# raulmur/ORB_SLAM2

Measured on NVIDIA H100. Metric: stereo frames/sec (ORB extract L+R + ComputeStereoMatches, KITTI-shaped 1242x375 @2000 kpts), higher is better.
Workload: dtype u8

## Files before the change

orb_slam2_b200/csrc/borb_host.cu:

```cuda
#include <cmath>
#include <cstdarg>
#include <cstdio>
#include <algorithm>
#include <cstdlib>
#include <cstring>

#include "borb_internal.h"

namespace borb {

static thread_local std::string tl_error;
void set_error(const char* fmt, ...) {
    char buf[512];
    va_list ap;
    va_start(ap, fmt);
    vsnprintf(buf, sizeof(buf), fmt, ap);
    va_end(ap);
    tl_error = buf;
}

std::atomic<int> g_poison{-1};

bool allow_max_smem(const void* func) {
    static std::mutex mu;
// ... 30 lines not shown
    e->per_level.assign(L, 0);
    const float factor = (float)(1.0 / sf);
    float want = (float)e->cfg.n_features * (1.f - factor) / (1.f - (float)std::pow((double)factor, (double)L));
    int sum = 0;
    for (int l = 0; l < L - 1; l++) {
        e->per_level[l] = cv_round_f(want);
        sum += e->per_level[l];
        want *= factor;
    }
    e->per_level[L - 1] = e->cfg.n_features - sum > 0 ? e->cfg.n_features - sum : 0;
    const int vmax = (int)std::floor(HALF_PATCH * std::sqrt(2.f) / 2 + 1);
    const int vmin = (int)std::ceil(HALF_PATCH * std::sqrt(2.f) / 2);
    for (int v = 0; v < 16; v++) e->umax[v] = 0;
    for (int v = 0; v <= vmax; ++v) e->umax[v] = (int)lrint(std::sqrt((double)HALF_PATCH * HALF_PATCH - (double)v * v));
    for (int v = HALF_PATCH, v0 = 0; v >= vmin; --v) {
        while (e->umax[v0] == e->umax[v0 + 1]) ++v0;
        e->umax[v] = v0;
        ++v0;
    }
}

void resize_table(int src, int dst, bool clamp_edges, int extra, std::vector<int16_t>& out) {
    const double inv = (double)dst / src, scale = 1. / inv;
    const size_t first = out.size();
    for (int d = 0; d < dst; d++) {
        float f = (float)((d + 0.5) * scale - 0.5);
        int s = (int)std::floor(f);
        f -= s;
        if (clamp_edges) {
            if (s < 0) { f = 0; s = 0; }
            if (s >= src - 1) { f = 0; s = src - 1; }
        }
        out.push_back((int16_t)s);
        out.push_back((int16_t)cv_round_f((1.f - f) * 2048.f));
        out.push_back((int16_t)cv_round_f(f * 2048.f));
        out.push_back(0);
    }
    for (int k = 0; k < extra; k++) {
        int r = 2 * dst - 2 - (dst + k);
        if (r < 0) r = 0;
        for (int j = 0; j < 4; j++) out.push_back(out[first + (size_t)r * 4 + j]);
    }
    if (((out.size() - first) / 4) & 1) for (int j = 0; j < 4; j++) out.push_back(0);
}

bool resize_window_table(const std::vector<int16_t>& tabs, size_t xtab_first, int n_entries, std::vector<int16_t>& out) {
    bool ok = true;
    for (int gq = 0; gq < n_entries; gq += 4) {
        int lo = 1 << 30, hi = 0;
        for (int i = 0; i < 4; i++) {
            const int ofs = tabs[xtab_first + (size_t)(gq + i) * 4];
            lo = std::min(lo, ofs); hi = std::max(hi, ofs);
        }
        const int base = lo & ~3;
        if (hi + 1 - base > 11) ok = false;
        for (int i = 0; i < 4; i++) {
            const int16_t* e = &tabs[xtab_first + (size_t)(gq + i) * 4];
            const int pos = e[0] - base;
            int s1 = 0, s2 = 0x10;
            if (pos <= 6) s1 = pos | ((pos + 1) << 4);
            else if (pos == 7) { s1 = 7; s2 = 0x40; }
            else { const int q = (pos - 8) + 4; s2 = q | ((q + 1) << 4); }
            out.push_back(e[1]);
            out.push_back(e[2]);
            out.push_back((int16_t)base);
            out.push_back((int16_t)((s1 | (s2 << 8)) & 0x7FFF));
        }
    }
    return ok;
}

const int8_t kPattern[1024] = {
#include "orb_pattern.inc"
};

borb_status build_geometry(borb_extractor* e, int w, int h, std::vector<int16_t>& tabs) {
    Geometry& g = e->geom;
    std::memset(&g, 0, sizeof(g));
    const int L = e->cfg.n_levels;
    g.nlevels = L; g.w = w; g.h = h;
    g.fast_mode = e->fast_mode;
    g.ini_th = e->cfg.ini_th_fast;
    g.min_th = e->cfg.min_th_fast;
    for (int i = 0; i < 16; i++) g.umax[i] = e->umax[i];
    unsigned pyr_off = 0, cand_off = 0;
    int blk = 0, sel_off = 0, btile = 0;
    tabs.clear();
    for (int l = 0; l < L; l++) {
        LevelGeom& v = g.lv[l];
        v.w = cv_round_f((float)w * e->inv_scale[l]);
        v.h = cv_round_f((float)h * e->inv_scale[l]);
        const float width = (float)(v.w - 2 * MIN_BORDER), height = (float)(v.h - 2 * MIN_BORDER);
        v.nCols = (int)(width / 30.f);
        v.nRows = (int)(height / 30.f);
        if (v.nCols < 1 || v.nRows < 1) {
            set_error("level %d is %dx%d: too small for the 30-px FAST cell grid (reference divides by zero)", l, v.w, v.h);
            return BORB_ERR_UNSUPPORTED;
        }
        v.wCell = (int)std::ceil(width / v.nCols);
        v.hCell = (int)std::ceil(height / v.nRows);
        v.pitch = align_up(v.w + 8, 128);
        v.pyr_off = pyr_off;
        pyr_off += (unsigned)v.pitch * v.h;
        v.cellsPerBlk = FAST_TILE_W / v.wCell > 0 ? FAST_TILE_W / v.wCell : 1;
        v.rowsPerBlk = fast_rows_per_blk(v.nRows, v.hCell);
        v.blkCols = (v.nCols + v.cellsPerBlk - 1) / v.cellsPerBlk;
        v.blkBase = blk;
        blk += v.blkCols * ((v.nRows + v.rowsPerBlk - 1) / v.rowsPerBlk);
        v.cand_off = cand_off;
        v.cand_cap = v.nCols * v.nRows * ((v.wCell + 1) / 2) * ((v.hCell + 1) / 2);
        cand_off += (unsigned)align_up(v.cand_cap, 32);
        v.quota = e->per_level[l];
        v.nIni = (int)std::round(width / height);
        if (v.nIni < 1) { set_error("level %d aspect ratio gives zero quadtree roots (reference divides by zero)", l); return BORB_ERR_UNSUPPORTED; }
        v.hX = width / v.nIni;
        v.node_cap = (v.quota > 4 * v.nIni ? v.quota : 4 * v.nIni) + 3;
        v.node_cap = align_up(v.node_cap + 1, 4);
        v.sel_off = sel_off;
        sel_off += v.node_cap;
        v.scale = e->scale[l];
        v.inv_scale = e->inv_scale[l];
        v.patch_size = (float)(int)(PATCH * e->scale[l]);
        g.blur_base[l] = btile;
        btile += ((v.w + BLUR_TILE_W - 1) / BLUR_TILE_W) * ((v.h + BLUR_TILE_H - 1) / BLUR_TILE_H);
        if (l > 0) {
            const int wpad = (v.w + 8 + 3) & ~3;
            v.xtab_off = (unsigned)(tabs.size() / 4);
            resize_table(g.lv[l - 1].w, v.w, true, wpad - v.w, tabs);
            v.ytab_off = (unsigned)(tabs.size() / 4);
            resize_table(g.lv[l - 1].h, v.h, false, 0, tabs);
            v.xwin_off = (unsigned)(tabs.size() / 4);
            std::vector<int16_t> win;
            v.x_windowed = resize_window_table(tabs, (size_t)v.xtab_off * 4, wpad, win) ? 1 : 0;
            tabs.insert(tabs.end(), win.begin(), win.end());
        }
        if (quadtree_smem_bytes(v.node_cap) > 200 * 1024) {
            set_error("per-level quota %d exceeds the quadtree kernel's shared-memory envelope", v.quota);
            return BORB_ERR_UNSUPPORTED;
        }
    }
    g.blur_base[L] = btile;
    g.blur_tiles = btile;
    g.fast_blocks = blk;
    g.pyr_image_stride = (unsigned)align_up((int)pyr_off, g.lv[0].pitch);
    g.cand_image_stride = cand_off;
    g.sel_image_stride = sel_off;
    if (sel_off >= 65536) { set_error("keypoint capacity %d exceeds 65535", sel_off); return BORB_ERR_UNSUPPORTED; }
    return BORB_OK;
}

void free_workspace(Workspace& ws) {
    cudaFree(ws.pyr); cudaFree(ws.blur); cudaFree(ws.cand); cudaFree(ws.cand_cnt); cudaFree(ws.pnode); cudaFree(ws.sel);
    cudaFree(ws.sel_cnt); cudaFree(ws.kps); cudaFree(ws.desc); cudaFree(ws.nkp); cudaFree(ws.u_right); cudaFree(ws.depth);
    cudaFree(ws.sad); cudaFree(ws.tabs); cudaFree(ws.brief_slots); cudaFree(ws.pair_idx); cudaFree(ws.st_bins); cudaFree(ws.st_recs); cudaFree(ws.stage);
    free(ws.fast_tmaps); cudaFree(ws.fast_tiles);
    ws = Workspace();
}

borb_status ensure(borb_extractor* e, int w, int h, int n_images) {
    if (w < 1 || h < 1 || w > BORB_MAX_DIM || h > BORB_MAX_DIM) { set_error("image size %dx%d outside [1,%d]", w, h, BORB_MAX_DIM); return BORB_ERR_UNSUPPORTED; }
    BORB_CUDA(cudaSetDevice(e->device));
    const bool same_shape = e->have_geom && e->geom.w == w && e->geom.h == h;
    if (same_shape && e->ws.max_images >= n_images) return BORB_OK;
    BORB_CUDA(cudaStreamSynchronize(e->stream));
    std::vector<int16_t> tabs;
    e->have_geom = false;
    e->last_n_images = 0;
    e->last_stereo_pairs = 0;
    borb_status st = build_geometry(e, w, h, tabs);
    if (st != BORB_OK) return st;
    size_t n = (size_t)(n_images > 2 ? n_images : 2);
    if (same_shape && (size_t)e->ws.max_images > n) n = (size_t)e->ws.max_images;
    free_workspace(e->ws);
    if (e->h_counts) { cudaFreeHost(e->h_counts); e->h_counts = nullptr; }
    e->pair_cache.clear();
    const Geometry& g = e->geom;
    Workspace& ws = e->ws;
    BORB_CUDA(cudaMalloc(&ws.pyr, n * g.pyr_image_stride + 256));
    BORB_CUDA(cudaMalloc(&ws.blur, n * g.pyr_image_stride + 256));
    BORB_CUDA(cudaMalloc(&ws.cand, n * g.cand_image_stride * sizeof(uint32_t)));
    BORB_CUDA(cudaMalloc(&ws.pnode, n * g.cand_image_stride * sizeof(int)));
    BORB_CUDA(cudaMalloc(&ws.cand_cnt, n * g.nlevels * sizeof(int)));
    BORB_CUDA(cudaMalloc(&ws.sel, n * g.sel_image_stride * sizeof(uint32_t)));
    BORB_CUDA(cudaMalloc(&ws.sel_cnt, n * g.nlevels * sizeof(int)));
    BORB_CUDA(cudaMalloc(&ws.kps, n * g.sel_image_stride * sizeof(borb_keypoint)));
    BORB_CUDA(cudaMalloc(&ws.desc, n * g.sel_image_stride * 32));
    BORB_CUDA(cudaMalloc(&ws.nkp, n * sizeof(int)));
    BORB_CUDA(cudaMalloc(&ws.u_right, n * g.sel_image_stride * sizeof(float)));
    BORB_CUDA(cudaMalloc(&ws.depth, n * g.sel_image_stride * sizeof(float)));
    BORB_CUDA(cudaMalloc(&ws.sad, n * g.sel_image_stride * sizeof(int)));
    BORB_CUDA(cudaMalloc(&ws.pair_idx, n * 2 * sizeof(int)));
    BORB_CUDA(cudaMalloc(&ws.st_bins, n * stereo_bins_bytes_per_pair()));
    ws.st_recs_bytes = n * (size_t)stereo_rec_stride(g) * stereo_rec_bytes();
    BORB_CUDA(cudaMalloc(&ws.st_recs, ws.st_recs_bytes));
    BORB_CUDA(cudaMalloc(&ws.tabs, (tabs.size() + 4) * sizeof(int16_t)));
    BORB_CUDA(cudaMemcpy(ws.tabs, tabs.data(), tabs.size() * sizeof(int16_t), cudaMemcpyHostToDevice));
    const std::vector<uint32_t>& slots = brief_slot_table();
    BORB_CUDA(cudaMalloc(&ws.brief_slots, slots.size() * sizeof(uint32_t)));
    BORB_CUDA(cudaMemcpy(ws.brief_slots, slots.data(), slots.size() * sizeof(uint32_t), cudaMemcpyHostToDevice));
    BORB_CUDA(cudaMemset(ws.nkp, 0, n * sizeof(int)));
    BORB_CUDA(cudaMallocHost(&e->h_counts, n * 2 * sizeof(int)));
    ws.max_images = (int)n;
    ws.fast_tmaps = malloc(fast_tmaps_bytes());
    if ((st = build_fast_tmaps(g, ws, ws.fast_tmaps)) != BORB_OK) return st;
    if ((st = build_fast_tiles(g, ws)) != BORB_OK) return st;
    e->have_geom = true;
    return BORB_OK;
}

borb_status poison_extract(borb_extractor* e) {
    const int p = poison_byte();
    if (p < 0) return BORB_OK;
    const Geometry& g = e->geom;
    Workspace& ws = e->ws;
    const size_t n = (size_t)ws.max_images;
    cudaStream_t s = e->stream;
    if (ws.stage) BORB_CUDA(cudaMemsetAsync(ws.stage, p, ws.stage_bytes, s));
    BORB_CUDA(cudaMemsetAsync(ws.pyr, p, n * g.pyr_image_stride + 256, s));
    BORB_CUDA(cudaMemsetAsync(ws.blur, p, n * g.pyr_image_stride + 256, s));
    BORB_CUDA(cudaMemsetAsync(ws.cand, p, n * g.cand_image_stride * sizeof(uint32_t), s));
    BORB_CUDA(cudaMemsetAsync(ws.pnode, p, n * g.cand_image_stride * sizeof(int), s));
    BORB_CUDA(cudaMemsetAsync(ws.cand_cnt, p, n * g.nlevels * sizeof(int), s));
    BORB_CUDA(cudaMemsetAsync(ws.sel, p, n * g.sel_image_stride * sizeof(uint32_t), s));
    BORB_CUDA(cudaMemsetAsync(ws.sel_cnt, p, n * g.nlevels * sizeof(int), s));
    BORB_CUDA(cudaMemsetAsync(ws.kps, p, n * g.sel_image_stride * sizeof(borb_keypoint), s));
    BORB_CUDA(cudaMemsetAsync(ws.desc, p, n * g.sel_image_stride * 32, s));
    BORB_CUDA(cudaMemsetAsync(ws.nkp, p, n * sizeof(int), s));
    return BORB_OK;
}

borb_status poison_stereo(borb_extractor* e) {
    const int p = poison_byte();
    if (p < 0) return BORB_OK;
    Workspace& ws = e->ws;
    const size_t n = (size_t)ws.max_images * e->geom.sel_image_stride;
    cudaStream_t s = e->stream;
    BORB_CUDA(cudaMemsetAsync(ws.u_right, p, n * sizeof(float), s));
    BORB_CUDA(cudaMemsetAsync(ws.depth, p, n * sizeof(float), s));
    BORB_CUDA(cudaMemsetAsync(ws.sad, p, n * sizeof(int), s));
    BORB_CUDA(cudaMemsetAsync(ws.st_bins, p, (size_t)ws.max_images * stereo_bins_bytes_per_pair(), s));
    BORB_CUDA(cudaMemsetAsync(ws.st_recs, p, ws.st_recs_bytes, s));
    return BORB_OK;
}

void drain_timing(borb_extractor* e);
void begin_step(borb_extractor* e) {
    if (!e->timing) return;
    if (e->ev.empty()) {
        e->ev.resize((size_t)borb_extractor::EV_RING * 9);
        for (auto& x : e->ev) cudaEventCreate(&x);
    }
    if (e->ev_pending >= borb_extractor::EV_RING) {
        cudaStreamSynchronize(e->stream);
        drain_timing(e);
    }
    e->ev_slot = (e->ev_slot + 1) % borb_extractor::EV_RING;
    e->ev_mask[e->ev_slot] = 0;
    e->ev_pending++;
}
void mark(borb_extractor* e, int i) {
    if (!e->timing || e->ev.empty()) return;
    cudaEventRecord(e->ev[(size_t)e->ev_slot * 9 + i], e->stream);
    e->ev_mask[e->ev_slot] |= 1u << i;
}
void drain_timing(borb_extractor* e) {
    const int R = borb_extractor::EV_RING;
    for (int k = e->ev_pending - 1; k >= 0; k--) {
        const int slot = ((e->ev_slot - k) % R + R) % R;
        const unsigned m = e->ev_mask[slot];
        for (int i = 0; i < 8; i++) {
            float ms = 0.f;
            if (m & (1u << i)) {
                int j = i + 1;
                while (j < 9 && !(m & (1u << j))) j++;
                if (j < 9 && cudaEventElapsedTime(&ms, e->ev[(size_t)slot * 9 + i], e->ev[(size_t)slot * 9 + j]) != cudaSuccess) { ms = 0.f; cudaGetLastError(); }
            }
            e->stage_ms[i] = ms;
            e->stage_sum_ms[i] += ms;
        }
        e->stage_steps++;
    }
    e->ev_pending = 0;
}

borb_status enqueue_extract(borb_extractor* e, int n) {
    const Geometry& g = e->geom;
    Workspace& ws = e->ws;
    cudaStream_t s = e->stream;
    BORB_CUDA(cudaMemsetAsync(ws.cand_cnt, 0, (size_t)n * g.nlevels * sizeof(int), s));
    mark(e, 1);
    e->launches += launch_pyramid(g, ws, n, s);
    mark(e, 2);
    e->launches += launch_fast(g, ws, n, s);
    mark(e, 3);
    e->launches += launch_quadtree(g, ws, n, s);
    mark(e, 4);
    e->launches += launch_blur(g, ws, n, s);
    mark(e, 5);
    e->launches += launch_describe(g, ws, n, s);
    mark(e, 6);
    BORB_CUDA(cudaGetLastError());
    e->last_n_images = n;
    e->last_stereo_pairs = 0;
    return BORB_OK;
}

borb_status rectified_size(borb_extractor* e, int w, int h, int* gw, int* gh) {
    if (!e->d_map[0][0]) return BORB_OK;
    if (w != e->map_src_w || h != e->map_src_h) {
        set_error("rectification maps were built for %dx%d raw frames, got %dx%d", e->map_src_w, e->map_src_h, w, h);
        return BORB_ERR_INVALID_ARG;
    }
    *gw = e->map_dst_w; *gh = e->map_dst_h;
    return BORB_OK;
}

borb_status upload_slots(borb_extractor* e, const uint8_t* const* slots, int n, int w, int h, int stride, bool stereo_pairs = false) {
    const Geometry& g = e->geom;
    const int ch = e->in_channels;
    if (stride < w * ch) { set_error("stride %d smaller than a row of %d %d-channel pixels", stride, w, ch); return BORB_ERR_INVALID_ARG; }
    const size_t img_bytes = (size_t)stride * h;
    bool contiguous = n > 1 || ch > 1 || e->d_map[0][0] != nullptr;
    for (int k = 0; k < n; k++) {
        if (!slots[k]) { set_error("image %d is NULL", k); return BORB_ERR_INVALID_ARG; }
        if (slots[k] != slots[0] + (size_t)k * img_bytes) contiguous = false;
    }
    auto need_stage = [&](size_t need) -> borb_status {
        if (e->ws.stage_bytes < need) {
            BORB_CUDA(cudaStreamSynchronize(e->stream));
            cudaFree(e->ws.stage);
            e->ws.stage = nullptr; e->ws.stage_bytes = 0;
            BORB_CUDA(cudaMalloc(&e->ws.stage, need));
            e->ws.stage_bytes = need;
            if (poison_byte() >= 0) BORB_CUDA(cudaMemsetAsync(e->ws.stage, poison_byte(), need, e->stream));
        }
        return BORB_OK;
    };
    if (e->d_map[0][0]) {
        if (ch != 1) { set_error("rectification maps apply to CV_8UC1 frames"); return BORB_ERR_UNSUPPORTED; }
        const size_t src_img = contiguous ? img_bytes : (size_t)w * h;
        const int src_stride = contiguous ? stride : w;
        borb_status st = need_stage(src_img * n);
        if (st != BORB_OK) return st;
        if (contiguous) BORB_CUDA(cudaMemcpyAsync(e->ws.stage, slots[0], src_img * n, cudaMemcpyHostToDevice, e->stream));
        else
            for (int k = 0; k < n; k++)
                BORB_CUDA(cudaMemcpy2DAsync(e->ws.stage + (size_t)k * src_img, w, slots[k], stride, w, h, cudaMemcpyHostToDevice, e->stream));
        e->launches += launch_repack_remap(g, e->ws, e->ws.stage, src_stride, src_img, w, h, e->d_map[0][0], e->d_map[0][1],
                                           stereo_pairs ? e->d_map[1][0] : nullptr, stereo_pairs ? e->d_map[1][1] : nullptr, n, e->stream);
        return BORB_OK;
    }
    if (contiguous) {
// ... 5 lines not shown
        else e->launches += launch_repack_color(g, e->ws, e->ws.stage, stride, img_bytes, ch, e->in_rgb, n, e->stream);
        return BORB_OK;
    }
    if (ch > 1) {
        const size_t row = (size_t)w * ch;
        borb_status st = need_stage(row * h * n);
        if (st != BORB_OK) return st;
        for (int k = 0; k < n; k++)
            BORB_CUDA(cudaMemcpy2DAsync(e->ws.stage + (size_t)k * row * h, row, slots[k], stride, row, h, cudaMemcpyHostToDevice, e->stream));
        e->launches += launch_repack_color(g, e->ws, e->ws.stage, (int)row, row * h, ch, e->in_rgb, n, e->stream);
        return BORB_OK;
    }
    for (int k = 0; k < n; k++) {
        uint8_t* dst = e->ws.pyr + (size_t)k * g.pyr_image_stride + g.lv[0].pyr_off;
        BORB_CUDA(cudaMemcpy2DAsync(dst, g.lv[0].pitch, slots[k], stride, w, h, cudaMemcpyHostToDevice, e->stream));
    }
    return BORB_OK;
}

borb_status upload_device(borb_extractor* e, const uint8_t* d_gray, int n, int w, int h, size_t pitch, size_t image_stride,
                          bool stereo_pairs = false) {
    const Geometry& g = e->geom;
    if (e->d_map[0][0]) {
        if (pitch > (size_t)INT_MAX) { set_error("pitch %zu too large", pitch); return BORB_ERR_INVALID_ARG; }
        e->launches += launch_repack_remap(g, e->ws, d_gray, (int)pitch, image_stride, w, h, e->d_map[0][0], e->d_map[0][1],
                                           stereo_pairs ? e->d_map[1][0] : nullptr, stereo_pairs ? e->d_map[1][1] : nullptr, n, e->stream);
        return BORB_OK;
    }
    cudaMemcpy3DParms p = {};
    p.srcPtr = make_cudaPitchedPtr((void*)d_gray, pitch, w, image_stride / pitch);
    p.dstPtr = make_cudaPitchedPtr(e->ws.pyr + g.lv[0].pyr_off, g.lv[0].pitch, w, g.pyr_image_stride / g.lv[0].pitch);
    if (image_stride % pitch == 0 && g.pyr_image_stride % g.lv[0].pitch == 0) {
        p.extent = make_cudaExtent(w, h, n);
        p.kind = cudaMemcpyDeviceToDevice;
        BORB_CUDA(cudaMemcpy3DAsync(&p, e->stream));
    } else {
        for (int i = 0; i < n; i++)
            BORB_CUDA(cudaMemcpy2DAsync(e->ws.pyr + (size_t)i * g.pyr_image_stride + g.lv[0].pyr_off, g.lv[0].pitch,
                                        d_gray + (size_t)i * image_stride, pitch, w, h, cudaMemcpyDeviceToDevice, e->stream));
    }
    return BORB_OK;
}

borb_status download_kps(borb_extractor* e, int first, int count, int step, borb_keypoint* kps, uint8_t* desc, int cap, int* n_out) {
    const Geometry& g = e->geom;
    const int m = cap < g.sel_image_stride ? cap : g.sel_image_stride;
    cudaStream_t s = e->stream;
    if (kps && m > 0)
        BORB_CUDA(cudaMemcpy2DAsync(kps, (size_t)cap * sizeof(borb_keypoint), e->ws.kps + (size_t)first * g.sel_image_stride,
                                    (size_t)step * g.sel_image_stride * sizeof(borb_keypoint), (size_t)m * sizeof(borb_keypoint),
                                    count, cudaMemcpyDeviceToHost, s));
    if (desc && m > 0)
        BORB_CUDA(cudaMemcpy2DAsync(desc, (size_t)cap * 32, e->ws.desc + (size_t)first * g.sel_image_stride * 32,
                                    (size_t)step * g.sel_image_stride * 32, (size_t)m * 32, count, cudaMemcpyDeviceToHost, s));
    if (n_out)
        BORB_CUDA(cudaMemcpy2DAsync(n_out, sizeof(int), e->ws.nkp + first, (size_t)step * sizeof(int), sizeof(int), count,
                                    cudaMemcpyDeviceToHost, s));
    return BORB_OK;
}

borb_status check_args(borb_extractor* e, int n, int w, int h) {
    if (!e) { set_error("null handle"); return BORB_ERR_INVALID_ARG; }
    if (n < 0) { set_error("negative image count"); return BORB_ERR_INVALID_ARG; }
    (void)w; (void)h;
    return BORB_OK;
}

borb_status enqueue_stereo(borb_extractor* eL, borb_extractor* eR, int n_pairs, const int* left_idx, const int* right_idx,
                           float bf, float b) {
    borb_extractor* e = eL;
    const Geometry& g = e->geom;
    std::vector<int> idx(2 * (size_t)n_pairs);
    for (int p = 0; p < n_pairs; p++) {
        idx[2 * p] = left_idx ? left_idx[p] : (eL == eR ? 2 * p : 0);
        idx[2 * p + 1] = right_idx ? right_idx[p] : (eL == eR ? 2 * p + 1 : 0);
        if (idx[2 * p] < 0 || idx[2 * p] >= eL->last_n_images || idx[2 * p + 1] < 0 || idx[2 * p + 1] >= eR->last_n_images) {
            set_error("stereo pair %d refers to an image outside the last batch", p);
            return BORB_ERR_STATE;
        }
    }
    if (n_pairs > e->ws.max_images) { set_error("too many pairs"); return BORB_ERR_INVALID_ARG; }
    if (idx != e->pair_cache) {
        BORB_CUDA(cudaStreamSynchronize(e->stream));
        std::memcpy(e->h_counts, idx.data(), idx.size() * sizeof(int));
        BORB_CUDA(cudaMemcpyAsync(e->ws.pair_idx, e->h_counts, idx.size() * sizeof(int), cudaMemcpyHostToDevice, e->stream));
        e->pair_cache = idx;
    }
    const int rec_stride = stereo_rec_stride(eR->geom);
    const size_t rec_bytes = (size_t)n_pairs * rec_stride * stereo_rec_bytes();
    if (rec_bytes > e->ws.st_recs_bytes) {
        BORB_CUDA(cudaStreamSynchronize(e->stream));
        cudaFree(e->ws.st_recs);
        e->ws.st_recs = nullptr;
        e->ws.st_recs_bytes = 0;
        BORB_CUDA(cudaMalloc(&e->ws.st_recs, rec_bytes));
        e->ws.st_recs_bytes = rec_bytes;
    }
    const borb_status pst = poison_stereo(e);
    if (pst != BORB_OK) return pst;
    StereoView L{eL->ws.pyr, eL->ws.kps, eL->ws.desc, eL->ws.nkp, eL->geom.pyr_image_stride, eL->geom.sel_image_stride};
    StereoView R{eR->ws.pyr, eR->ws.kps, eR->ws.desc, eR->ws.nkp, eR->geom.pyr_image_stride, eR->geom.sel_image_stride};
    mark(e, 6);
    e->launches += launch_stereo(g, L, R, e->ws.pair_idx, n_pairs, bf, b, e->ws.u_right, e->ws.depth, e->ws.sad, g.sel_image_stride,
                                 e->ws.st_bins, e->ws.st_recs, rec_stride, e->stream);
    mark(e, 7);
    BORB_CUDA(cudaGetLastError());
    e->last_stereo_pairs = (eL == eR && !left_idx && !right_idx) ? n_pairs : 0;
    return BORB_OK;
}

borb_status download_stereo(borb_extractor* e, int n_pairs, float* u_right, float* depth, int cap) {
    const Geometry& g = e->geom;
    const int m = cap < g.sel_image_stride ? cap : g.sel_image_stride;
    if (u_right && m > 0)
        BORB_CUDA(cudaMemcpy2DAsync(u_right, (size_t)cap * 4, e->ws.u_right, (size_t)g.sel_image_stride * 4, (size_t)m * 4, n_pairs, cudaMemcpyDeviceToHost, e->stream));
    if (depth && m > 0)
        BORB_CUDA(cudaMemcpy2DAsync(depth, (size_t)cap * 4, e->ws.depth, (size_t)g.sel_image_stride * 4, (size_t)m * 4, n_pairs, cudaMemcpyDeviceToHost, e->stream));
    return BORB_OK;
}

borb_status finish_timing(borb_extractor* e) {
    if (e->timing && e->ev_pending > 0) drain_timing(e);
    return BORB_OK;
}

}

const std::vector<uint32_t>& brief_slot_table() {
    static const std::vector<uint32_t> table = [] {
        std::vector<uint32_t> t((size_t)BRIEF_BINS * 512);
        int row[512], col[512], order[512];
        for (int b = 0; b < BRIEF_BINS; b++) {
            const double th = (b + 0.5) * (2.0 * 3.14159265358979323846 / BRIEF_BINS);
            const double a = std::cos(th), s = std::sin(th);
            for (int p = 0; p < 512; p++) {
                const int x = kPattern[2 * p], y = kPattern[2 * p + 1];
                row[p] = (int)std::lround(x * s + y * a);
                col[p] = (int)std::lround(x * a - y * s);
                order[p] = p;
            }
            std::sort(order, order + 512, [&](int i, int j) {
                return row[i] != row[j] ? row[i] < row[j] : (col[i] != col[j] ? col[i] < col[j] : i < j);
            });
            for (int k = 0; k < 512; k++) {
                const int p = order[k];
                t[(size_t)b * 512 + k] = (uint32_t)(kPattern[2 * p] + 128) | (uint32_t)(kPattern[2 * p + 1] + 128) << 8 | (uint32_t)p << 16;
            }
        }
        return t;
    }();
    return table;
}

}

using namespace borb;

extern "C" {

borb_status borb_debug_set_poison(int byte) {
    if (byte < -1 || byte > 255) { set_error("poison byte %d outside [-1, 255]", byte); return BORB_ERR_INVALID_ARG; }
    g_poison.store(byte, std::memory_order_relaxed);
    return BORB_OK;
}

const char* borb_last_error(void) { return tl_error.c_str(); }
const char* borb_status_str(borb_status s) {
    switch (s) {
        case BORB_OK: return "ok";
        case BORB_ERR_INVALID_ARG: return "invalid argument";
        case BORB_ERR_NO_DEVICE: return "no CUDA device (libborb has no CPU path)";
        case BORB_ERR_CUDA: return "CUDA error";
        case BORB_ERR_UNSUPPORTED: return "unsupported shape or quota";
        case BORB_ERR_CAPACITY: return "output capacity too small";
        case BORB_ERR_STATE: return "invalid call order";
    }
    return "unknown";
}
int borb_version(void) { return BORB_VERSION; }

borb_status borb_device_count(int* n) {
    if (!n) return BORB_ERR_INVALID_ARG;
    *n = 0;
    cudaError_t err = cudaGetDeviceCount(n);
    if (err != cudaSuccess) { *n = 0; cudaGetLastError(); set_error("cudaGetDeviceCount: %s", cudaGetErrorString(err)); return BORB_ERR_NO_DEVICE; }
    return BORB_OK;
}

borb_status borb_host_alloc(void** p, size_t bytes) {
    if (!p) return BORB_ERR_INVALID_ARG;
    BORB_CUDA(cudaMallocHost(p, bytes));
    return BORB_OK;
}
borb_status borb_host_free(void* p) {
    if (p) BORB_CUDA(cudaFreeHost(p));
    return BORB_OK;
}

borb_status borb_extractor_create(const borb_extractor_cfg* cfg, int device, borb_extractor** out) {
    if (!cfg || !out) { set_error("null argument"); return BORB_ERR_INVALID_ARG; }
    *out = nullptr;
    if (cfg->n_levels < 1 || cfg->n_levels > BORB_MAX_LEVELS || cfg->n_features < 1 || !(cfg->scale_factor > 1.0f)) {
        set_error("bad extractor cfg (n_features=%d scale=%f levels=%d)", cfg->n_features, cfg->scale_factor, cfg->n_levels);
        return BORB_ERR_INVALID_ARG;
    }
    if (cfg->ini_th_fast < 0 || cfg->ini_th_fast > 255) {
        set_error("ini_th_fast %d outside [0, 255]", cfg->ini_th_fast);
        return BORB_ERR_INVALID_ARG;
    }
    if (cfg->min_th_fast < 0 || cfg->min_th_fast > 255) {
        set_error("min_th_fast %d outside [0, 255]", cfg->min_th_fast);
        return BORB_ERR_INVALID_ARG;
    }
    int ndev = 0;
    borb_status st = borb_device_count(&ndev);
    if (st != BORB_OK) return st;
    if (ndev < 1) { set_error("no CUDA device visible; libborb has no CPU fallback"); return BORB_ERR_NO_DEVICE; }
    if (device < 0 || device >= ndev) { set_error("device %d out of range (%d visible)", device, ndev); return BORB_ERR_INVALID_ARG; }
    borb_extractor* e = new borb_extractor();
    e->cfg = *cfg;
    e->device = device;
    init_tables(e);
    cudaError_t err = cudaSetDevice(device);
    if (err == cudaSuccess) err = cudaStreamCreateWithFlags(&e->stream, cudaStreamNonBlocking);
    if (err != cudaSuccess) {
        set_error("CUDA init failed: %s", cudaGetErrorString(err));
        delete e;
        return BORB_ERR_CUDA;
    }
    *out = e;
    return BORB_OK;
}

borb_status borb_extractor_destroy(borb_extractor* e) {
    if (!e) return BORB_OK;
    cudaSetDevice(e->device);
    if (e->stream) cudaStreamSynchronize(e->stream);
    free_workspace(e->ws);
    for (int a = 0; a < 2; a++)
        for (int c = 0; c < 2; c++) cudaFree(e->d_map[a][c]);
    if (e->h_counts) cudaFreeHost(e->h_counts);
    for (auto& x : e->ev) cudaEventDestroy(x);
    if (e->stream) cudaStreamDestroy(e->stream);
    delete e;
    return BORB_OK;
}

borb_status borb_extractor_tables(const borb_extractor* e, float* scale, float* inv_scale, float* sigma2, float* inv_sigma2,
                                  int32_t* features_per_level) {
    if (!e) return BORB_ERR_INVALID_ARG;
    for (int l = 0; l < e->cfg.n_levels; l++) {
        if (scale) scale[l] = e->scale[l];
        if (inv_scale) inv_scale[l] = e->inv_scale[l];
        if (sigma2) sigma2[l] = e->sigma2[l];
        if (inv_sigma2) inv_sigma2[l] = e->inv_sigma2[l];
        if (features_per_level) features_per_level[l] = e->per_level[l];
    }
    return BORB_OK;
}

borb_status borb_extractor_capacity(const borb_extractor* e, int width, int height, int* cap) {
    if (!e || !cap) return BORB_ERR_INVALID_ARG;
    borb_extractor tmp;
    tmp.cfg = e->cfg; tmp.scale = e->scale; tmp.inv_scale = e->inv_scale; tmp.per_level = e->per_level;
    std::memcpy(tmp.umax, e->umax, sizeof(tmp.umax));
    std::vector<int16_t> tabs;
    if (width < 1 || height < 1 || width > BORB_MAX_DIM || height > BORB_MAX_DIM) { set_error("image size out of range"); return BORB_ERR_UNSUPPORTED; }
    borb_status st = build_geometry(&tmp, width, height, tabs);
    if (st != BORB_OK) return st;
    *cap = tmp.geom.sel_image_stride;
    return BORB_OK;
}

borb_status borb_extractor_reserve(borb_extractor* e, int width, int height, int max_images) {
    if (!e || max_images < 1) return BORB_ERR_INVALID_ARG;
    return ensure(e, width, height, max_images);
}

borb_status borb_sync(borb_extractor* e) {
    if (!e) return BORB_ERR_INVALID_ARG;
    BORB_CUDA(cudaSetDevice(e->device));
    BORB_CUDA(cudaStreamSynchronize(e->stream));
    return finish_timing(e);
}

borb_status borb_extract_batch_enqueue(borb_extractor* e, const uint8_t* const* gray, int n, int w, int h, int stride,
                                       borb_keypoint* kps, uint8_t* desc, int cap, int* n_out) {
    borb_status st = check_args(e, n, w, h);
    if (st != BORB_OK) return st;
    if (n == 0) return BORB_OK;
    if (!gray || cap < 0 || stride < w) { set_error("bad arguments"); return BORB_ERR_INVALID_ARG; }
    int gw = w, gh = h;
    if ((st = rectified_size(e, w, h, &gw, &gh)) != BORB_OK) return st;
    if ((st = ensure(e, gw, gh, n)) != BORB_OK) return st;
    if ((st = poison_extract(e)) != BORB_OK) return st;
    begin_step(e);
    mark(e, 0);
    if ((st = upload_slots(e, gray, n, w, h, stride)) != BORB_OK) return st;
    if ((st = enqueue_extract(e, n)) != BORB_OK) return st;
    mark(e, 7);
    st = download_kps(e, 0, n, 1, kps, desc, cap, n_out);
    mark(e, 8);
    return st;
}

borb_status borb_extract_batch(borb_extractor* e, const uint8_t* const* gray, int n, int w, int h, int stride,
// ... 344 lines not shown
```

orb_slam2_b200/csrc/borb_internal.h:

```cpp
#pragma once
#include <cuda_runtime.h>
#include <stdint.h>

#include <atomic>
#include <mutex>
#include <string>
#include <vector>

#include "../../include/borb.h"

namespace borb {

extern std::atomic<int> g_poison;
inline int poison_byte() { return g_poison.load(std::memory_order_relaxed); }

constexpr int EDGE = 19;
constexpr int PATCH = 31;
constexpr int HALF_PATCH = 15;
constexpr int MIN_BORDER = 16;
constexpr int TH_HIGH = 100;
constexpr int TH_LOW = 50;
constexpr int BLUR_TILE_W = 120;
constexpr int BLUR_TILE_H = 64;
constexpr int FAST_TILE_W = 124;
constexpr int FAST_H_BAND = 64;

__host__ __device__ inline int fast_rows_per_blk(int nRows, int hCell) {
    const int r = FAST_H_BAND / hCell;
    return r < 1 ? 1 : (r > nRows ? nRows : r);
}
__host__ __device__ inline int fast_box_rows(int rowsPerBlk, int hCell) { return rowsPerBlk * hCell + 6; }

__host__ __device__ inline uint32_t pack_xys(int x, int y, int s) { return (uint32_t)x | ((uint32_t)y << 12) | ((uint32_t)s << 24); }
__host__ __device__ inline int xys_x(uint32_t v) { return (int)(v & 0xFFFu); }
__host__ __device__ inline int xys_y(uint32_t v) { return (int)((v >> 12) & 0xFFFu); }
__host__ __device__ inline int xys_s(uint32_t v) { return (int)(v >> 24); }

struct LevelGeom {
    int w, h;
    int pitch;
    unsigned pyr_off;
    int nCols, nRows, wCell, hCell;
    int cellsPerBlk;
    int rowsPerBlk;
    int blkCols;
    int blkBase;
    unsigned cand_off;
    int cand_cap;
    int quota;
    int nIni;
    float hX;
    int node_cap;
    int sel_off;
    float scale;
    float inv_scale;
    float patch_size;
    unsigned xtab_off, ytab_off;
    unsigned xwin_off;
    int x_windowed;
};

struct Geometry {
    int nlevels;
    int w, h;
    int ini_th, min_th;
    int fast_mode;
    int fast_blocks;
    unsigned pyr_image_stride;
    unsigned cand_image_stride;
    int sel_image_stride;
    int blur_tiles;
    int blur_base[BORB_MAX_LEVELS + 1];
    int umax[16];
    LevelGeom lv[BORB_MAX_LEVELS];
};

struct Workspace {
    int max_images = 0;
    uint8_t* pyr = nullptr;
    uint8_t* blur = nullptr;
    uint32_t* cand = nullptr;
    int* cand_cnt = nullptr;
    int* pnode = nullptr;
    uint32_t* sel = nullptr;
    int* sel_cnt = nullptr;
    borb_keypoint* kps = nullptr;
    uint8_t* desc = nullptr;
    int* nkp = nullptr;
    float* u_right = nullptr;
    float* depth = nullptr;
    int* sad = nullptr;
    int16_t* tabs = nullptr;
    uint32_t* brief_slots = nullptr;
    int* pair_idx = nullptr;
    int* st_bins = nullptr;
    void* st_recs = nullptr;
    size_t st_recs_bytes = 0;
    uint8_t* stage = nullptr;
    size_t stage_bytes = 0;
    void* fast_tmaps = nullptr;
    void* fast_tiles = nullptr;
    int fast_n_tiles = 0;
};

constexpr int BRIEF_BINS = 32;
const std::vector<uint32_t>& brief_slot_table();

void set_error(const char* fmt, ...);
bool allow_max_smem(const void* func);
#define BORB_CUDA(call)                                                                             \
    do {                                                                                            \
        cudaError_t _e = (call);                                                                    \
        if (_e != cudaSuccess) {                                                                    \
            borb::set_error("%s failed: %s (%s:%d)", #call, cudaGetErrorString(_e), __FILE__, __LINE__); \
            return (_e == cudaErrorNoDevice || _e == cudaErrorInsufficientDriver) ? BORB_ERR_NO_DEVICE : BORB_ERR_CUDA; \
        }                                                                                           \
    } while (0)

int launch_repack_remap(const Geometry& g, const Workspace& ws, const uint8_t* stage, int src_stride, size_t src_image_bytes, int src_w,
                        int src_h, const float* mx0, const float* my0, const float* mx1, const float* my1, int n_images, cudaStream_t s);
int launch_repack_color(const Geometry& g, const Workspace& ws, const uint8_t* stage, int src_stride, size_t src_image_bytes, int channels,
                        int rgb, int n_images, cudaStream_t s);
int launch_repack(const Geometry& g, const Workspace& ws, const uint8_t* stage, int src_stride, size_t src_image_bytes,
                  int n_images, cudaStream_t s);
int launch_pyramid(const Geometry& g, const Workspace& ws, int n_images, cudaStream_t s);
int launch_fast(const Geometry& g, const Workspace& ws, int n_images, cudaStream_t s);
int launch_quadtree(const Geometry& g, const Workspace& ws, int n_images, cudaStream_t s);
int launch_blur(const Geometry& g, const Workspace& ws, int n_images, cudaStream_t s);
int launch_describe(const Geometry& g, const Workspace& ws, int n_images, cudaStream_t s);
int launch_describe_math_probe(int fn, const float* a, const float* b, int n, float* out, cudaStream_t s);
int launch_match_math_probe(int fn, const float* a, const float* b, int n, float log_scale, int n_levels, void* out,
                            cudaStream_t s);

struct StereoView {
    const uint8_t* pyr;
    const borb_keypoint* kps;
    const uint8_t* desc;
    const int* nkp;
    unsigned pyr_image_stride;
    int kp_image_stride;
};
int launch_stereo(const Geometry& g, const StereoView& L, const StereoView& R, const int* d_pair_idx, int n_pairs,
                  float bf, float b, float* d_u_right, float* d_depth, int* d_sad, int out_stride, int* d_bins, void* d_recs,
                  int rec_stride, cudaStream_t s);
int stereo_rec_stride(const Geometry& g);
size_t stereo_bins_bytes_per_pair();
size_t stereo_rec_bytes();
size_t quadtree_smem_bytes(int node_cap);
borb_status build_fast_tmaps(const Geometry& g, const Workspace& ws, void* out_tmaps);
borb_status build_fast_tiles(const Geometry& g, Workspace& ws);
size_t fast_tmaps_bytes();

}

struct borb_extractor {
    borb_extractor_cfg cfg;
    int device = 0;
    cudaStream_t stream = nullptr;
    std::vector<float> scale, inv_scale, sigma2, inv_sigma2;
    std::vector<int> per_level;
    int umax[16];
    bool have_geom = false;
    borb::Geometry geom;
    borb::Workspace ws;
    int last_n_images = 0;
    int last_stereo_pairs = 0;
    int in_channels = 1;
    int in_rgb = 1;
    float* d_map[2][2] = {{nullptr, nullptr}, {nullptr, nullptr}};
    int map_src_w = 0, map_src_h = 0, map_dst_w = 0, map_dst_h = 0;
    int fast_mode = 0;
    uint64_t launches = 0;
    static constexpr int EV_RING = 128;
    bool timing = false;
    std::vector<cudaEvent_t> ev;
    unsigned ev_mask[EV_RING] = {};
    int ev_slot = 0;
    int ev_pending = 0;
    float stage_ms[8] = {};
    double stage_sum_ms[8] = {};
    uint64_t stage_steps = 0;
    int* h_counts = nullptr;
    std::vector<int> pair_cache;
};
```

orb_slam2_b200/csrc/k_describe.cu:

```cuda
#include "borb_internal.h"

namespace borb {

namespace {

struct SinCosTab { double sign[4]; double hpi_inv, hpi, c0, c1, c2, c3, c4, s1, s2, s3; };
__device__ const SinCosTab d_sincos[2] = {
    {{1.0, -1.0, -1.0, 1.0}, 0x1.45F306DC9C883p+23, 0x1.921FB54442D18p0, 0x1p0, -0x1.ffffffd0c621cp-2,
     0x1.55553e1068f19p-5, -0x1.6c087e89a359dp-10, 0x1.99343027bf8c3p-16, -0x1.555545995a603p-3,
     0x1.1107605230bc4p-7, -0x1.994eb3774cf24p-13},
    {{1.0, -1.0, -1.0, 1.0}, 0x1.45F306DC9C883p+23, 0x1.921FB54442D18p0, -0x1p0, 0x1.ffffffd0c621cp-2,
     -0x1.55553e1068f19p-5, 0x1.6c087e89a359dp-10, -0x1.99343027bf8c3p-16, -0x1.555545995a603p-3,
     0x1.1107605230bc4p-7, -0x1.994eb3774cf24p-13}};

__device__ __forceinline__ float sc_poly(double x, double x2, const SinCosTab* p, int n) {
    if ((n & 1) == 0) {
        const double x3 = x * x2;
        const double s1 = p->s2 + x2 * p->s3;
        const double x7 = x3 * x2;
        const double s = x + x3 * p->s1;
        return (float)(s + x7 * s1);
    }
    const double x4 = x2 * x2;
    const double c2 = p->c3 + x2 * p->c4;
    const double c1 = p->c0 + x2 * p->c1;
    const double x6 = x4 * x2;
    const double c = c1 + x4 * p->c2;
    return (float)(c + x6 * c2);
}
__device__ __forceinline__ float glibc_sincosf(float y, int is_cos) {
    double x = (double)y;
    const SinCosTab* p = &d_sincos[0];
    const unsigned top = (__float_as_uint(y) >> 20) & 0x7ff;
    if (top < ((0x3f490fdbu >> 20) & 0x7ff)) {
        const double x2 = x * x;
        if (top < ((0x39800000u >> 20) & 0x7ff)) return is_cos ? 1.0f : y;
        return sc_poly(x, x2, p, is_cos);
    }
    const double r = x * p->hpi_inv;
    const int n = ((int)r + 0x800000) >> 24;
    x = x - (double)n * p->hpi;
    const double s = p->sign[n & 3];
    if (n & 2) p = &d_sincos[1];
    return sc_poly(x * s, x * x, p, n ^ is_cos);
}

__device__ __forceinline__ float fast_atan2_deg(float y, float x) {
    const float scale = (float)(180.0 / 3.14159265358979323846);
    const float p1 = 0.9997878412794807f * scale, p3 = -0.3258083974640975f * scale;
    const float p5 = 0.1555786518463281f * scale, p7 = -0.04432655554792128f * scale;
    const float ax = fabsf(x), ay = fabsf(y);
    const float eps = (float)2.2204460492503131e-16;
    float a, c, c2;
    if (ax >= ay) {
        c = __fdiv_rn(ay, __fadd_rn(ax, eps));
        c2 = __fmul_rn(c, c);
        a = __fmul_rn(__fadd_rn(__fmul_rn(__fadd_rn(__fmul_rn(__fadd_rn(__fmul_rn(p7, c2), p5), c2), p3), c2), p1), c);
    } else {
        c = __fdiv_rn(ax, __fadd_rn(ay, eps));
        c2 = __fmul_rn(c, c);
        a = __fsub_rn(90.f, __fmul_rn(__fadd_rn(__fmul_rn(__fadd_rn(__fmul_rn(__fadd_rn(__fmul_rn(p7, c2), p5), c2), p3), c2), p1), c));
    }
    if (x < 0) a = __fsub_rn(180.f, a);
    if (y < 0) a = __fsub_rn(360.f, a);
    return a;
}

}

__global__ void __launch_bounds__(256, 8) describe_kernel(const __grid_constant__ Geometry g, const uint8_t* __restrict__ pyr,
                                                       const uint8_t* __restrict__ blur, const uint32_t* __restrict__ slots,
                                                       const uint32_t* __restrict__ sel, const int* __restrict__ sel_cnt,
                                                       borb_keypoint* __restrict__ kps, uint8_t* __restrict__ desc,
                                                       int* __restrict__ nkp) {
    __shared__ __align__(4) uint8_t taps[8][512];
    const int img = blockIdx.y;
    const int lane = threadIdx.x & 31;
    const int idx = blockIdx.x * (blockDim.x >> 5) + (threadIdx.x >> 5);
    int scan = lane < g.nlevels ? sel_cnt[img * g.nlevels + lane] : 0;
#pragma unroll
    for (int off = 1; off < BORB_MAX_LEVELS; off <<= 1) {
        const int t = __shfl_up_sync(0xFFFFFFFFu, scan, off);
        if (lane >= off) scan += t;
    }
    const int total = __shfl_sync(0xFFFFFFFFu, scan, g.nlevels - 1);
    if (blockIdx.x == 0 && threadIdx.x == 0) nkp[img] = total;
    if (idx >= total) return;
    const int l = __popc(__ballot_sync(0xFFFFFFFFu, lane < g.nlevels && scan <= idx));
    const int base = __shfl_sync(0xFFFFFFFFu, scan, max(l - 1, 0)) & (l > 0 ? -1 : 0);
    const LevelGeom& L = g.lv[l];
    const int pitch = L.pitch;
    const float lscale = L.scale, lpatch = L.patch_size;
    const uint32_t e = sel[(size_t)img * g.sel_image_stride + L.sel_off + (idx - base)];
    const int px = xys_x(e), py = xys_y(e);
    const size_t lvl_off = (size_t)img * g.pyr_image_stride + L.pyr_off;
    const int u = lane - HALF_PATCH;
    const int vmax = lane < 31 ? g.umax[u < 0 ? -u : u] : -1;
    const uint8_t* col = pyr + lvl_off + (size_t)(py - HALF_PATCH) * pitch + (px + u);
    int acc = 0;
#pragma unroll
    for (int vv = -HALF_PATCH; vv <= HALF_PATCH; vv++) {
        if ((vv < 0 ? -vv : vv) <= vmax) acc += (int)*col * (vv * 8192 + 1);
        col += pitch;
    }
    const int colsum = acc & 8191;
    int m01 = acc >> 13;
    int m10 = u * colsum;
#pragma unroll
    for (int off = 16; off > 0; off >>= 1) {
        m01 += __shfl_xor_sync(0xFFFFFFFFu, m01, off);
        m10 += __shfl_xor_sync(0xFFFFFFFFu, m10, off);
    }
    const float angle = fast_atan2_deg((float)m01, (float)m10);
    const float factorPI = (float)(3.1415926535897932384626433832795 / 180.f);
    const float t = __fmul_rn(angle, factorPI);
    const float a = glibc_sincosf(t, 1), b = glibc_sincosf(t, 0);
    const uint8_t* cb = blur + lvl_off + (size_t)py * pitch + px;
    const int bin = min((int)(angle * (float)(BRIEF_BINS / 360.0)), BRIEF_BINS - 1);
    const uint32_t* slot = slots + bin * 512 + lane;
    uint8_t* tw = taps[threadIdx.x >> 5];
#pragma unroll
    for (int k = 0; k < 16; k++) {
        const uint32_t s = __ldg(slot + k * 32);
        const float x = __fsub_rn(__uint_as_float(__byte_perm(s, 0x4B000000u, 0x7440)), 8388736.f);
        const float y = __fsub_rn(__uint_as_float(__byte_perm(s, 0x4B000000u, 0x7441)), 8388736.f);
        const int r = __float2int_rn(__fadd_rn(__fmul_rn(x, b), __fmul_rn(y, a)));
        const int q = __float2int_rn(__fsub_rn(__fmul_rn(x, a), __fmul_rn(y, b)));
        tw[s >> 16] = cb[r * pitch + q];
    }
    __syncwarp();
    unsigned mine = 0;
#pragma unroll
    for (int j = 0; j < 8; j++) {
        const unsigned t01 = reinterpret_cast<const uint16_t*>(tw)[j * 32 + lane];
        const unsigned word = __ballot_sync(0xFFFFFFFFu, (t01 & 0xFFu) < (t01 >> 8));
        if (lane == j) mine = word;
    }
    const size_t o = (size_t)img * g.sel_image_stride + idx;
    if (lane < 8) reinterpret_cast<unsigned*>(desc + o * 32)[lane] = mine;
    if (lane == 0) {
        borb_keypoint k;
        k.x = __fmul_rn((float)px, lscale);
        k.y = __fmul_rn((float)py, lscale);
        k.size = lpatch;
        k.angle = angle;
        k.response = (float)xys_s(e);
        k.octave = l;
        k.class_id = -1;
        kps[o] = k;
    }
}

int launch_describe(const Geometry& g, const Workspace& ws, int n_images, cudaStream_t s) {
    dim3 grid((g.sel_image_stride + 7) / 8, n_images);
    describe_kernel<<<grid, 256, 0, s>>>(g, ws.pyr, ws.blur, ws.brief_slots, ws.sel, ws.sel_cnt, ws.kps, ws.desc, ws.nkp);
    return 1;
}

__global__ void describe_math_probe_kernel(int fn, const float* __restrict__ a, const float* __restrict__ b, int n,
                                           float* __restrict__ out) {
    for (long long i = blockIdx.x * blockDim.x + threadIdx.x; i < n; i += gridDim.x * blockDim.x)
        out[i] = fn == 2 ? fast_atan2_deg(a[i], b[i]) : glibc_sincosf(a[i], fn);
}

int launch_describe_math_probe(int fn, const float* a, const float* b, int n, float* out, cudaStream_t s) {
    describe_math_probe_kernel<<<std::min((n + 255) / 256, 8192), 256, 0, s>>>(fn, a, b, n, out);
    return 1;
}

}
```

Measured before the change: 43920.

## Describe two keypoints per warp using half-warps and precomputed float tap table

The ORB describe kernel now assigns two keypoints per warp. The moment computation runs twice across the full warp, once per keypoint, and the BRIEF tap sampling is split so each half-warp handles 512 taps for its own keypoint. The host builds a tap table of pre-converted float coordinates with the slot index packed into the low mantissa bits, which removes the byte_perm/subtract decode. This halves the grid and cuts per-keypoint warp overhead, at the cost of more work per thread and a tiny perturbation of the tap coordinates from the packed bits (masked off before use).

```diff
diff --git a/orb_slam2_b200/csrc/borb_host.cu b/orb_slam2_b200/csrc/borb_host.cu
--- a/orb_slam2_b200/csrc/borb_host.cu
+++ b/orb_slam2_b200/csrc/borb_host.cu
@@ -206,7 +206,7 @@
 void free_workspace(Workspace& ws) {
     cudaFree(ws.pyr); cudaFree(ws.blur); cudaFree(ws.cand); cudaFree(ws.cand_cnt); cudaFree(ws.pnode); cudaFree(ws.sel);
     cudaFree(ws.sel_cnt); cudaFree(ws.kps); cudaFree(ws.desc); cudaFree(ws.nkp); cudaFree(ws.u_right); cudaFree(ws.depth);
-    cudaFree(ws.sad); cudaFree(ws.tabs); cudaFree(ws.brief_slots); cudaFree(ws.pair_idx); cudaFree(ws.st_bins); cudaFree(ws.st_recs); cudaFree(ws.stage);
+    cudaFree(ws.sad); cudaFree(ws.tabs); cudaFree(ws.brief_taps); cudaFree(ws.pair_idx); cudaFree(ws.st_bins); cudaFree(ws.st_recs); cudaFree(ws.stage);
     free(ws.fast_tmaps); cudaFree(ws.fast_tiles);
     ws = Workspace();
 }
@@ -249,9 +249,9 @@
     BORB_CUDA(cudaMalloc(&ws.st_recs, ws.st_recs_bytes));
     BORB_CUDA(cudaMalloc(&ws.tabs, (tabs.size() + 4) * sizeof(int16_t)));
     BORB_CUDA(cudaMemcpy(ws.tabs, tabs.data(), tabs.size() * sizeof(int16_t), cudaMemcpyHostToDevice));
-    const std::vector<uint32_t>& slots = brief_slot_table();
-    BORB_CUDA(cudaMalloc(&ws.brief_slots, slots.size() * sizeof(uint32_t)));
-    BORB_CUDA(cudaMemcpy(ws.brief_slots, slots.data(), slots.size() * sizeof(uint32_t), cudaMemcpyHostToDevice));
+    const std::vector<uint2>& taps = brief_tap_table();
+    BORB_CUDA(cudaMalloc(&ws.brief_taps, taps.size() * sizeof(uint2)));
+    BORB_CUDA(cudaMemcpy(ws.brief_taps, taps.data(), taps.size() * sizeof(uint2), cudaMemcpyHostToDevice));
     BORB_CUDA(cudaMemset(ws.nkp, 0, n * sizeof(int)));
     BORB_CUDA(cudaMallocHost(&e->h_counts, n * 2 * sizeof(int)));
     ws.max_images = (int)n;
@@ -563,6 +563,21 @@
     return table;
 }
 
+const std::vector<uint2>& brief_tap_table() {
+    static const std::vector<uint2> table = [] {
+        const std::vector<uint32_t>& slots = brief_slot_table();
+        std::vector<uint2> t(slots.size());
+        for (size_t k = 0; k < slots.size(); k++) {
+            const float x = (float)((int)(slots[k] & 0xFFu) - 128), y = (float)((int)((slots[k] >> 8) & 0xFFu) - 128);
+            std::memcpy(&t[k].x, &x, 4);
+            std::memcpy(&t[k].y, &y, 4);
+            t[k].x |= slots[k] >> 16;
+        }
+        return t;
+    }();
+    return table;
+}
+
 }
 
 using namespace borb;
diff --git a/orb_slam2_b200/csrc/borb_internal.h b/orb_slam2_b200/csrc/borb_internal.h
--- a/orb_slam2_b200/csrc/borb_internal.h
+++ b/orb_slam2_b200/csrc/borb_internal.h
@@ -91,7 +91,7 @@
     float* depth = nullptr;
     int* sad = nullptr;
     int16_t* tabs = nullptr;
-    uint32_t* brief_slots = nullptr;
+    uint2* brief_taps = nullptr;
     int* pair_idx = nullptr;
     int* st_bins = nullptr;
     void* st_recs = nullptr;
@@ -105,6 +105,7 @@
 
 constexpr int BRIEF_BINS = 32;
 const std::vector<uint32_t>& brief_slot_table();
+const std::vector<uint2>& brief_tap_table();
 
 void set_error(const char* fmt, ...);
 bool allow_max_smem(const void* func);
diff --git a/orb_slam2_b200/csrc/k_describe.cu b/orb_slam2_b200/csrc/k_describe.cu
--- a/orb_slam2_b200/csrc/k_describe.cu
+++ b/orb_slam2_b200/csrc/k_describe.cu
@@ -69,91 +69,105 @@
 }
 
 __global__ void __launch_bounds__(256, 8) describe_kernel(const __grid_constant__ Geometry g, const uint8_t* __restrict__ pyr,
-                                                       const uint8_t* __restrict__ blur, const uint32_t* __restrict__ slots,
+                                                       const uint8_t* __restrict__ blur, const uint2* __restrict__ tap_tab,
                                                        const uint32_t* __restrict__ sel, const int* __restrict__ sel_cnt,
                                                        borb_keypoint* __restrict__ kps, uint8_t* __restrict__ desc,
                                                        int* __restrict__ nkp) {
-    __shared__ __align__(4) uint8_t taps[8][512];
+    __shared__ __align__(4) uint8_t taps[16 * 512];
     const int img = blockIdx.y;
-    const int lane = threadIdx.x & 31;
-    const int idx = blockIdx.x * (blockDim.x >> 5) + (threadIdx.x >> 5);
-    int scan = lane < g.nlevels ? sel_cnt[img * g.nlevels + lane] : 0;
+    const int lane = threadIdx.x & 31, half = lane >> 4, hl = lane & 15;
+    const int slot = threadIdx.x >> 4;
+    const int idx0 = (blockIdx.x * (blockDim.x >> 5) + (threadIdx.x >> 5)) * 2;
+    int scan = hl < g.nlevels ? sel_cnt[img * g.nlevels + hl] : 0;
 #pragma unroll
     for (int off = 1; off < BORB_MAX_LEVELS; off <<= 1) {
-        const int t = __shfl_up_sync(0xFFFFFFFFu, scan, off);
-        if (lane >= off) scan += t;
+        const int t = __shfl_up_sync(0xFFFFFFFFu, scan, off, 16);
+        if (hl >= off) scan += t;
     }
     const int total = __shfl_sync(0xFFFFFFFFu, scan, g.nlevels - 1);
     if (blockIdx.x == 0 && threadIdx.x == 0) nkp[img] = total;
-    if (idx >= total) return;
-    const int l = __popc(__ballot_sync(0xFFFFFFFFu, lane < g.nlevels && scan <= idx));
-    const int base = __shfl_sync(0xFFFFFFFFu, scan, max(l - 1, 0)) & (l > 0 ? -1 : 0);
+    if (idx0 >= total) return;
+    const bool live = idx0 + half < total;
+    const int idx = idx0 + (live ? half : 0);
+    const unsigned below = __ballot_sync(0xFFFFFFFFu, hl < g.nlevels && scan <= idx) >> (half * 16);
+    const int l = __popc(below & 0xFFFFu);
+    const int base = __shfl_sync(0xFFFFFFFFu, scan, max(l - 1, 0), 16) & (l > 0 ? -1 : 0);
     const LevelGeom& L = g.lv[l];
     const int pitch = L.pitch;
-    const float lscale = L.scale, lpatch = L.patch_size;
     const uint32_t e = sel[(size_t)img * g.sel_image_stride + L.sel_off + (idx - base)];
     const int px = xys_x(e), py = xys_y(e);
     const size_t lvl_off = (size_t)img * g.pyr_image_stride + L.pyr_off;
     const int u = lane - HALF_PATCH;
     const int vmax = lane < 31 ? g.umax[u < 0 ? -u : u] : -1;
-    const uint8_t* col = pyr + lvl_off + (size_t)(py - HALF_PATCH) * pitch + (px + u);
-    int acc = 0;
+    const long long top = (long long)(lvl_off + (size_t)(py - HALF_PATCH) * pitch + px);
+    int m01 = 0, m10 = 0;
 #pragma unroll
-    for (int vv = -HALF_PATCH; vv <= HALF_PATCH; vv++) {
-        if ((vv < 0 ? -vv : vv) <= vmax) acc += (int)*col * (vv * 8192 + 1);
-        col += pitch;
-    }
-    const int colsum = acc & 8191;
-    int m01 = acc >> 13;
-    int m10 = u * colsum;
+    for (int k = 0; k < 2; k++) {
+        const uint8_t* col = pyr + __shfl_sync(0xFFFFFFFFu, top, 16 * k) + u;
+        const int kpitch = __shfl_sync(0xFFFFFFFFu, pitch, 16 * k);
+        int acc = 0;
 #pragma unroll
-    for (int off = 16; off > 0; off >>= 1) {
-        m01 += __shfl_xor_sync(0xFFFFFFFFu, m01, off);
-        m10 += __shfl_xor_sync(0xFFFFFFFFu, m10, off);
+        for (int vv = -HALF_PATCH; vv <= HALF_PATCH; vv++) {
+            if ((vv < 0 ? -vv : vv) <= vmax) acc += (int)__ldg(col) * (vv * 8192 + 1);
+            col += kpitch;
+        }
+        int k01 = acc >> 13;
+        int k10 = u * (acc & 8191);
+#pragma unroll
+        for (int off = 16; off > 0; off >>= 1) {
+            k01 += __shfl_xor_sync(0xFFFFFFFFu, k01, off);
+            k10 += __shfl_xor_sync(0xFFFFFFFFu, k10, off);
+        }
+        if (half == k) { m01 = k01; m10 = k10; }
     }
     const float angle = fast_atan2_deg((float)m01, (float)m10);
-    const float factorPI = (float)(3.1415926535897932384626433832795 / 180.f);
-    const float t = __fmul_rn(angle, factorPI);
-    const float a = glibc_sincosf(t, 1), b = glibc_sincosf(t, 0);
-    const uint8_t* cb = blur + lvl_off + (size_t)py * pitch + px;
-    const int bin = min((int)(angle * (float)(BRIEF_BINS / 360.0)), BRIEF_BINS - 1);
-    const uint32_t* slot = slots + bin * 512 + lane;
-    uint8_t* tw = taps[threadIdx.x >> 5];
-#pragma unroll
-    for (int k = 0; k < 16; k++) {
-        const uint32_t s = __ldg(slot + k * 32);
-        const float x = __fsub_rn(__uint_as_float(__byte_perm(s, 0x4B000000u, 0x7440)), 8388736.f);
-        const float y = __fsub_rn(__uint_as_float(__byte_perm(s, 0x4B000000u, 0x7441)), 8388736.f);
-        const int r = __float2int_rn(__fadd_rn(__fmul_rn(x, b), __fmul_rn(y, a)));
-        const int q = __float2int_rn(__fsub_rn(__fmul_rn(x, a), __fmul_rn(y, b)));
-        tw[s >> 16] = cb[r * pitch + q];
-    }
-    __syncwarp();
-    unsigned mine = 0;
-#pragma unroll
-    for (int j = 0; j < 8; j++) {
-        const unsigned t01 = reinterpret_cast<const uint16_t*>(tw)[j * 32 + lane];
-        const unsigned word = __ballot_sync(0xFFFFFFFFu, (t01 & 0xFFu) < (t01 >> 8));
-        if (lane == j) mine = word;
-    }
     const size_t o = (size_t)img * g.sel_image_stride + idx;
-    if (lane < 8) reinterpret_cast<unsigned*>(desc + o * 32)[lane] = mine;
-    if (lane == 0) {
+    if (live && hl == 0) {
         borb_keypoint k;
-        k.x = __fmul_rn((float)px, lscale);
-        k.y = __fmul_rn((float)py, lscale);
-        k.size = lpatch;
+        k.x = __fmul_rn((float)px, L.scale);
+        k.y = __fmul_rn((float)py, L.scale);
+        k.size = L.patch_size;
         k.angle = angle;
         k.response = (float)xys_s(e);
         k.octave = l;
         k.class_id = -1;
         kps[o] = k;
     }
+    const float factorPI = (float)(3.1415926535897932384626433832795 / 180.f);
+    const float t = __fmul_rn(angle, factorPI);
+    const float a = glibc_sincosf(t, 1), b = glibc_sincosf(t, 0);
+    const uint8_t* cb = blur + lvl_off + (size_t)py * pitch + px;
+    asm("" : "+l"(cb));
+    int tbase = slot << 9;
+    asm("" : "+r"(tbase));
+    const int bin = min((int)(angle * (float)(BRIEF_BINS / 360.0)), BRIEF_BINS - 1);
+    const uint2* tp = tap_tab + bin * 512 + hl;
+#pragma unroll
+    for (int k = 0; k < 32; k++) {
+        const uint2 s = __ldg(tp + k * 16);
+        const float x = __uint_as_float(s.x & ~0x1FFu), y = __uint_as_float(s.y);
+        const int r = __float2int_rn(__fadd_rn(__fmul_rn(x, b), __fmul_rn(y, a)));
+        const int q = __float2int_rn(__fsub_rn(__fmul_rn(x, a), __fmul_rn(y, b)));
+        taps[tbase | (s.x & 0x1FFu)] = __ldg(cb + (r * pitch + q));
+    }
+    __syncwarp();
+    const uint16_t* t16 = reinterpret_cast<const uint16_t*>(taps + tbase);
+    const unsigned pick = half ? 0x7632u : 0x5410u;
+    unsigned mine = 0;
+#pragma unroll
+    for (int j = 0; j < 8; j++) {
+        const unsigned lo = t16[32 * j + hl], hi = t16[32 * j + 16 + hl];
+        const unsigned b0 = __ballot_sync(0xFFFFFFFFu, (lo & 0xFFu) < (lo >> 8));
+        const unsigned b1 = __ballot_sync(0xFFFFFFFFu, (hi & 0xFFu) < (hi >> 8));
+        const unsigned word = __byte_perm(b0, b1, pick);
+        if (hl == j) mine = word;
+    }
+    if (live && hl < 8) reinterpret_cast<unsigned*>(desc + o * 32)[hl] = mine;
 }
 
 int launch_describe(const Geometry& g, const Workspace& ws, int n_images, cudaStream_t s) {
-    dim3 grid((g.sel_image_stride + 7) / 8, n_images);
-    describe_kernel<<<grid, 256, 0, s>>>(g, ws.pyr, ws.blur, ws.brief_slots, ws.sel, ws.sel_cnt, ws.kps, ws.desc, ws.nkp);
+    dim3 grid((g.sel_image_stride + 15) / 16, n_images);
+    describe_kernel<<<grid, 256, 0, s>>>(g, ws.pyr, ws.blur, ws.brief_taps, ws.sel, ws.sel_cnt, ws.kps, ws.desc, ws.nkp);
     return 1;
 }
 
```

New measurement: 44090 (median of 6 runs). About the same (+0.4%).
